# OpenDriveLab/ViDAR

Measured on AMD Instinct MI355X. Metric: train samples/sec (6-cam->BEV step), higher is better.
Workload: dtype f32

## Files before the change

### include/vidar_hip.h

```cpp
#ifndef VIDAR_HIP_H_
#define VIDAR_HIP_H_

#include <stddef.h>
#include <stdint.h>

#ifdef __cplusplus
extern "C" {
#endif

#define VIDAR_ERR_BAD_ARG (-22)

int vidar_abi_version(void);
int vidar_marker(int id, void* stream);

int vidar_set_deterministic(int on);
int vidar_get_deterministic(void);

int vidar_dvr_max_d(void);

int vidar_dvr_render_forward_f32(const float* sigma, const float* origin, const float* points,
                                 const float* tindex, float* pred_dist ,
                                 float* gt_dist , int N, int M, int T, int TO, int Z, int Y,
                                 int X, int train_phase, void* stream);

// ... 175 lines not shown
                            void* workspace, size_t workspace_bytes, void* stream);
int vidar_ray_occupancy_cam_f32(const float* sigma, const float* pix2vox, float* hit, float* free_,
                                int F, int C, int Hs, int Ws, float u0, float v0, float du, float dv,
                                int Z, int Y, int X, int K, float step,
                                void* workspace, size_t workspace_bytes, void* stream);

#define VIDAR_GEMM_F32 0
#define VIDAR_GEMM_BF16X3 1
#define VIDAR_GEMM_K_MAJOR 0
#define VIDAR_GEMM_MN_MAJOR 1
int vidar_gemm_f32(const float* A, int64_t lda, int a_layout, const float* B, int64_t ldb, int b_layout, float* C,
                   int64_t ldc, int M, int N, int K, int batch, int64_t strideA, int64_t strideB, int64_t strideC,
                   const float* scale, const float* shift, int vec_axis, const float* residual, int64_t ldr,
                   int64_t strideR, int relu, int precision, int reduce, float* a_rowsum, void* workspace,
                   size_t workspace_bytes, void* stream);
int vidar_gemm_splits(int M, int N, int K, int batch, int precision, int reduce);
size_t vidar_gemm_workspace_bytes(int M, int N, int K, int batch, int precision, int reduce);
int vidar_gemm_set_variant(int variant);

int vidar_dcn_set_variant(int variant);
int vidar_dcn_im2col_f32(const float* x, const float* offset, const float* mask, float* cols, int N,
                         int C, int H, int W, int Ho, int Wo, int kh, int kw, int stride, int pad,
                         int dil, void* stream);
int vidar_dcn_col2im_det_workspace_bytes(int N, int C, int H, int W, int64_t* bytes);
int vidar_dcn_col2im_f32(const float* grad_cols, const float* x, const float* offset,
                         const float* mask, float* grad_x, float* grad_offset, float* grad_mask,
                         int N, int C, int H, int W, int Ho, int Wo, int kh, int kw, int stride,
                         int pad, int dil, void* workspace, size_t workspace_bytes, void* stream);
size_t vidar_dcn_col2im_workspace_bytes(int N, int H, int W, int Ho, int Wo, int kh, int kw);

// ... 65 lines not shown
```

### vidar_amd/_lib.py

```python
from __future__ import annotations

import ctypes
import os
from pathlib import Path

_PKG = Path(__file__).resolve().parent
LIB_PATH = _PKG / "libvidar_hip.so"
_lib = None
BAD_ARG = -22


class VidarHipError(RuntimeError):
    pass


def lib() -> ctypes.CDLL:
    global _lib
    if _lib is None:
        import torch
        if not LIB_PATH.exists():
            raise VidarHipError(
                f"{LIB_PATH} not found: build it with `python -m vidar_amd.build` "
                f"(or __graft_entry__.build()); vidar_amd has no CPU fallback")
        _lib = declare(ctypes.CDLL(str(LIB_PATH)))
# ... 65 lines not shown
    "vidar_ray_gumbel_fwd_f32": "i 7p 6i f p",
    "vidar_ray_gumbel_bwd_f32": "i 7p 6i f p z p",
    "vidar_ray_argmax_f32": "i 6p 6i f p",
    "vidar_ray_dist_fwd_f32": "i 9p 6i f p",
    "vidar_ray_dist_bwd_f32": "i 7p 6i f p z p",
    "vidar_ray_max_k": "i",
    "vidar_ray_force_streamed": "i i",
    "vidar_ray_argmax_cam_f32": "i 3p 4i 4f 4i f p",
    "vidar_cam_rays_f32": "i 3p 4i 4f p",
    "vidar_ray_stats_f32": "i 7p 6i f p",
    "vidar_ray_stats_cam_f32": "i 4p 4i 4f 4i f p",
    "vidar_ray_occupancy_workspace_bytes": "i 4i p",
    "vidar_ray_occupancy_f32": "i 6p 6i f p z p",
    "vidar_ray_occupancy_cam_f32": "i 4p 4i 4f 4i f p z p",
    "vidar_gemm_f32": "i p l i p l i p l 4i 3l 2p i p 2l 3i 2p z p",
    "vidar_gemm_splits": "i 6i",
    "vidar_gemm_workspace_bytes": "z 6i",
    "vidar_gemm_set_variant": "i i",
    "vidar_dcn_set_variant": "i i",
    "vidar_dcn_im2col_f32": "i 4p 11i p",
    "vidar_dcn_col2im_f32": "i 7p 11i p z p",
    "vidar_dcn_col2im_workspace_bytes": "z 7i",
    "vidar_dcn_col2im_det_workspace_bytes": "i 4i p",
    "vidar_conv3x3_few_workspace_bytes": "z i",
    "vidar_conv3x3_few_f32": "i 4p 5i p z p",
    "vidar_affine_act_fwd_f32": "i 5p 4i p",
    "vidar_stem_bn_relu_pool_f32": "i 4p 4i p",
    "vidar_affine_act_bwd_f32": "i 5p 4i p",
    "vidar_dcnv3_set_variant": "i i",
    "vidar_dcnv3_forward_f32": "i 4p 13i f p",
# ... 107 lines not shown
```

### vidar_amd/csrc/gemm_mfma.hip

```cpp
#include <hip/hip_runtime.h>

#include <stdint.h>

#include <type_traits>

#include "vidar_hip.h"
#include "vidar_common.h"

namespace {

typedef __bf16 bf16x8 __attribute__((ext_vector_type(8)));
typedef __bf16 bf16x2 __attribute__((ext_vector_type(2)));
typedef float f32x16 __attribute__((ext_vector_type(16)));
typedef float f32x2 __attribute__((ext_vector_type(2)));
typedef float f32x4 __attribute__((ext_vector_type(4)));
typedef float f32x4u __attribute__((ext_vector_type(4), aligned(4)));
typedef uint32_t u32x4 __attribute__((ext_vector_type(4)));
typedef uint32_t u32x2 __attribute__((ext_vector_type(2)));

constexpr int BM = 128, BN = 128, THREADS = 256;
constexpr int BK = 32;
constexpr int MN_STRIDE = 128 + 8;
template <int PREC>
struct Geo {
// ... 6 lines not shown
constexpr int LAY_K = 0, LAY_MN = 1;

struct GemmArgs {
  const float* A; const float* B; float* C;
  int64_t lda, ldb, ldc, sA, sB, sC;
  int M, N, K;
  int splits, k_chunk;
  int slabs;
  const float* scale; const float* shift; int vec_axis;
  const float* residual; int64_t ldr, sR;
  int relu;
  int tiles_m, tiles_n, m_fastest;
  int total;
  float* a_rowsum;
  float* rowsum_ws;
};

struct Lane {
  int wm, wn, l31, h;
  __device__ __forceinline__ Lane(int tid, int wave) : wm((wave >> 1) * 64), wn((wave & 1) * 64), l31(tid & 31), h((tid & 63) >> 5) {}
  __device__ __forceinline__ explicit Lane(int tid) : Lane(tid, tid >> 6) {}
  __device__ __forceinline__ uint32_t voff(uint32_t ld) const { return (uint32_t)(((wm + 4 * h) * ld + wn + l31) * 4); }
};

__device__ __forceinline__ void zero_acc(f32x16 (&acc)[2][2]) {
#pragma unroll
  for (int i = 0; i < 2; ++i)
#pragma unroll
    for (int j = 0; j < 2; ++j)
#pragma unroll
      for (int r = 0; r < 16; ++r) acc[i][j][r] = 0.0f;
// ... 103 lines not shown
      *(u32x4*)(img + u * MN_STRIDE + cq) = hi;
      *(u32x4*)(img + Geo<PREC>::IMG_DWORDS + u * MN_STRIDE + cq) = lo;
    }
  } else {
#pragma unroll
    for (int i = 0; i < 4; ++i) {
      const int item = tid + 256 * i;
      *(u32x4*)(img + (item >> 5) * MN_STRIDE + (item & 31) * 4) = __builtin_bit_cast(u32x4, s.v[i >> 1][i & 1]);
    }
  }
}
template <int PREC, int ALAY, int BLAY>
__device__ __forceinline__ void stage_pair(const Staged& sa, const Staged& sb, uint32_t* imgA, uint32_t* imgB, int tid) {
  stage<PREC, ALAY>(sa, imgA, tid);
  stage<PREC, BLAY>(sb, imgB, tid);
}

template <int PREC, int LAY>
__device__ __forceinline__ u32x4 frag(const uint32_t* img, int row, int s, int h) {
  if (LAY == LAY_K) {
    if (PREC == PREC_BF16X3)
      return *(const u32x4*)(img + row * Geo<PREC>::KM_STRIDE + (((2 * s + h) ^ ((row >> 2) & 3)) << 2));
    return *(const u32x4*)(img + row * Geo<PREC>::KM_STRIDE + 8 * s + 4 * h);
  }
  u32x4 f;
  const uint32_t* p = img + (8 * s + 4 * h) * MN_STRIDE + row;
#pragma unroll
  for (int j = 0; j < 4; ++j) f[j] = p[j * MN_STRIDE];
  return f;
}
// ... 70 lines not shown
          }
    } else {
#pragma unroll
      for (int u = 0; u < 4; ++u)
#pragma unroll
        for (int i = 0; i < 2; ++i)
#pragma unroll
          for (int j = 0; j < 2; ++j) {
            const f32x4 bf = __builtin_bit_cast(f32x4, fb[j][0]), af = __builtin_bit_cast(f32x4, fa[i][0]);
            acc[i][j] = __builtin_amdgcn_mfma_f32_32x32x2f32(af[u], bf[u], acc[i][j], 0, 0, 0);
          }
    }
  }
}

template <int PREC, int ALAY, int BLAY>
__device__ __forceinline__ void mainloop(f32x16 (&acc)[2][2], Staged& sa, Staged& sb, const GemmArgs& g, const Tile& T,
                                         int kstop, uint32_t* imgA, uint32_t* imgB, int tid, uint32_t voa, uint32_t vob,
                                         f32x4& rowsum, bool want_rowsum) {
  const Lane c(tid);
  for (int k0 = T.kbeg; k0 < kstop; k0 += BK) {
    if (ALAY == LAY_MN && want_rowsum) add_rowsum(rowsum, sa);
    stage_pair<PREC, ALAY, BLAY>(sa, sb, imgA, imgB, tid);
    __syncthreads();
    if (k0 + BK < T.kend) fetch<PREC, ALAY, BLAY>(sa, sb, g, T, k0 + BK, tid, voa, vob);
    mma_step<PREC, ALAY, BLAY>(acc, imgA, imgB, c);
    __syncthreads();
  }
}

__device__ __forceinline__ float finish(float acc, float sc, float sh, float rs, int relu) {
  float y = acc * sc + sh + rs;
  if (relu && !(y > 0.0f)) y = 0.0f;
  return y;
}

template <bool RAGGED_M>
__device__ __forceinline__ void epilogue_impl(const f32x16 (&acc)[2][2], const GemmArgs& g, const Tile& T, int tid) {
  const Lane c(tid);
  const int m0 = T.m0, n0 = T.n0;
  float* C; int64_t ldc;
  if (g.slabs) { C = g.C + (int64_t)T.z * g.M * g.N; ldc = g.N; }
  else { C = g.C + (int64_t)T.batch * g.sC; ldc = g.ldc; }
  const bool epi = !g.slabs;
  const bool by_n = epi && g.vec_axis == 0, by_m = epi && g.vec_axis == 1;
  const int rows_left = g.M - m0, cols_left = g.N - n0;
  const int mleft = rows_left - c.wm - 4 * c.h;
  const __amdgpu_buffer_rsrc_t rsC = window_rsrc(C + (int64_t)m0 * ldc + n0, ldc, rows_left, cols_left);
  const uint32_t voC = c.voff((uint32_t)ldc);
  const bool has_res = epi && g.residual != nullptr;
  const float* Rp = has_res ? g.residual + (int64_t)T.batch * g.sR + (int64_t)m0 * g.ldr + n0 : C;
  const __amdgpu_buffer_rsrc_t rsR = window_rsrc(Rp, g.ldr, rows_left, cols_left, has_res);
// ... 13 lines not shown
    for (int i = 0; i < 2; ++i) {
#pragma unroll
      for (int r0 = 0; r0 < 16; r0 += 8) {
        float sc[8], sh[8], rs[8];
#pragma unroll
        for (int r = 0; r < 8; ++r) {
          const int row = 32 * i + (r & 3) + 8 * ((r0 + r) >> 2);
          sc[r] = m_scale ? ld4(rsS, voM, (uint32_t)(row * 4)) : sn;
          sh[r] = m_shift ? ld4(rsH, voM, (uint32_t)(row * 4)) : bn;
          rs[r] = has_res ? ld4(rsR, voR, (uint32_t)((row * (uint32_t)g.ldr + 32 * j) * 4)) : 0.0f;
        }
#pragma unroll
        for (int r = 0; r < 8; ++r) {
          const int row = 32 * i + (r & 3) + 8 * ((r0 + r) >> 2);
          float y = acc[i][j][r0 + r];
          if (epi) y = finish(y, sc[r], sh[r], rs[r], g.relu);
          if (!RAGGED_M || row < mleft)
            __builtin_amdgcn_raw_buffer_store_b32(__builtin_bit_cast(uint32_t, y), rsC, voC,
                                                    (uint32_t)((row * (uint32_t)ldc + 32 * j) * 4), 0);
        }
      }
    }
  }
}

__device__ __forceinline__ void epilogue(const f32x16 (&acc)[2][2], const GemmArgs& g, const Tile& T, int tid) {
  if (g.M - T.m0 >= BM) epilogue_impl<false>(acc, g, T, tid);
  else epilogue_impl<true>(acc, g, T, tid);
}

constexpr int TAB_DWORDS = 2 * (BM + BM);

__device__ __forceinline__ void lds_barrier() { asm volatile("s_waitcnt lgkmcnt(0)\n\ts_barrier" ::: "memory"); }

__device__ __forceinline__ bool piped_tile(const GemmArgs& g, const Tile& T) {
  return !g.slabs && (g.vec_axis == 1 || (g.scale == nullptr && g.shift == nullptr)) && g.M - T.m0 >= BM &&
         g.N - T.n0 >= BN && T.kbeg < T.kend;
}

__device__ __forceinline__ float table_value(const GemmArgs& g, const Tile& T, int tid) {
  const float* v = tid < BM ? g.scale : g.shift;
  float x = tid < BM ? 1.0f : 0.0f;
  if (v != nullptr) x = v[T.m0 + (tid & (BM - 1))];
  return x;
}

template <int ALAY, int BLAY>
__device__ __forceinline__ void last_step_stage(const Staged& sa, const Staged& sb, uint32_t* imgA, uint32_t* imgB,
                                                float* tab, float tabv, int tid) {
  stage_pair<PREC_F32, ALAY, BLAY>(sa, sb, imgA, imgB, tid);
  tab[tid] = tabv;
  __syncthreads();
}

template <int ALAY, int BLAY>
__device__ __forceinline__ void last_step_piped(f32x16 (&acc)[2][2], const GemmArgs& g, const Tile& T, const uint32_t* imgA,
                                                const uint32_t* imgB, const float* tab, int tid0) {
  constexpr int PREC = PREC_F32;
  int tid = tid0;
  asm volatile("" : "+v"(tid));
  const Lane c(tid);
  const __amdgpu_buffer_rsrc_t rsC =
      window_rsrc(g.C + (int64_t)T.batch * g.sC + (int64_t)T.m0 * g.ldc + T.n0, g.ldc, BM, BN);
  const uint32_t ldc = (uint32_t)g.ldc, ldr = (uint32_t)g.ldr;
// ... 26 lines not shown
        if (sub < 4) acc[i][j] = __builtin_amdgcn_mfma_f32_32x32x2f32(af[u], bf[u], acc[i][j], 0, 0, 0);
        if (sub > 0) {
          const int r = 4 * s + u;
          const int prow = 32 * pi + 8 * s + u;
          const float y = finish(acc[pi][pj][r], tsc[prow], tsh[prow], rs[r], g.relu);
          __builtin_amdgcn_raw_buffer_store_b32(__builtin_bit_cast(uint32_t, y), rsC, voC, (uint32_t)((prow * ldc + 32 * pj) * 4), 0);
          if (sub < 4) rs[r] = ld4(rsR, voRz, (uint32_t)(((32 * i + 8 * s + u) * ldr + 32 * j) * rb));
        }
      }
      __builtin_amdgcn_sched_barrier(0);
    }
    if (sub == 3) lds_barrier();
  }
}

template <int PREC, int ALAY, int BLAY>
__global__ __launch_bounds__(THREADS, 3) void gemm_mfma_kernel(GemmArgs g) {
  constexpr int IMGS = (PREC == PREC_BF16X3) ? 2 : 1;
  constexpr int IMGS_DWORDS = 2 * IMGS * Geo<PREC>::IMG_DWORDS;
  __shared__ __attribute__((aligned(16))) uint32_t lds[IMGS_DWORDS + (PREC == PREC_F32 && ALAY == LAY_K ? TAB_DWORDS : 0)];
  uint32_t* imgA = lds;
  uint32_t* imgB = lds + IMGS * Geo<PREC>::IMG_DWORDS;
  const int tid = threadIdx.x;
  const uint32_t voa = voff<PREC, ALAY>(g.lda, tid), vob = voff<PREC, BLAY>(g.ldb, tid);
  Staged sa, sb;
  int t = blockIdx.x;
  if (t >= g.total) return;
  Tile cur = decode_tile<PREC, ALAY, BLAY>(g, t);
  if (cur.kbeg < cur.kend) fetch<PREC, ALAY, BLAY>(sa, sb, g, cur, cur.kbeg, tid, voa, vob);
  for (int parity = 0;; parity ^= 1) {
    f32x16 acc[2][2];
    zero_acc(acc);
    f32x4 rowsum = {0.f, 0.f, 0.f, 0.f};
    const bool want_rowsum = ALAY == LAY_MN && g.a_rowsum != nullptr && cur.n0 == 0;
    const int tn = t + (int)gridDim.x;
    const bool more = tn < g.total;
    constexpr bool PIPED = PREC == PREC_F32 && ALAY == LAY_K;
    const bool piped = PIPED && piped_tile(g, cur);
    float tabv = 0.0f;
    if (piped) tabv = table_value(g, cur, tid);
    const int kstop = piped ? cur.kbeg + (cur.kend - cur.kbeg - 1) / BK * BK : cur.kend;
    mainloop<PREC, ALAY, BLAY>(acc, sa, sb, g, cur, kstop, imgA, imgB, tid, voa, vob, rowsum, want_rowsum);
    float* tab = reinterpret_cast<float*>(lds) + IMGS_DWORDS + parity * (TAB_DWORDS / 2);
    if constexpr (PIPED) {
      if (piped) last_step_stage<ALAY, BLAY>(sa, sb, imgA, imgB, tab, tabv, tid);
    }
    if (want_rowsum) {
      float* red = reinterpret_cast<float*>(lds);
      const int quad = tid & 31, part = tid >> 5;
      *(f32x4*)(red + (part * 32 + quad) * 4) = rowsum;
      __syncthreads();
      if (tid < BM) {
        float sum = 0.f;
#pragma unroll
        for (int p8 = 0; p8 < 8; ++p8) sum += red[(p8 * 32 + (tid >> 2)) * 4 + (tid & 3)];
        if (cur.m0 + tid < g.M) g.rowsum_ws[(int64_t)cur.z * g.M + cur.m0 + tid] = sum;
      }
      __syncthreads();
    }
    if (more) {
      const Tile nxt = decode_tile<PREC, ALAY, BLAY>(g, tn);
      if (nxt.kbeg < nxt.kend) fetch<PREC, ALAY, BLAY>(sa, sb, g, nxt, nxt.kbeg, tid, voa, vob);
    }
    if constexpr (PIPED) {
      if (piped) last_step_piped<ALAY, BLAY>(acc, g, cur, imgA, imgB, tab, tid);
      else epilogue(acc, g, cur, tid);
    } else {
      epilogue(acc, g, cur, tid);
    }
    if (!more) break;
    cur = decode_tile<PREC, ALAY, BLAY>(g, tn);
    t = tn;
  }
}

constexpr int WS_THREADS = 512;

template <int PREC, int ALAY, int BLAY>
struct Cursor {
  int t;
  int k0;
  Tile T;
  __device__ __forceinline__ void start(const GemmArgs& g, int t0) {
// ... 108 lines not shown
}

int g_gemm_variant = 0;

template <class F>
void with_layouts(int a_layout, int b_layout, F f) {
  using K = std::integral_constant<int, LAY_K>;
  using MN = std::integral_constant<int, LAY_MN>;
  if (a_layout == LAY_K && b_layout == LAY_K) f(K{}, K{});
  else if (a_layout == LAY_K) f(K{}, MN{});
  else if (b_layout == LAY_K) f(MN{}, K{});
  else f(MN{}, MN{});
}

template <int PREC>
void launch(const GemmArgs& g, int a_layout, int b_layout, bool ws, int grid, hipStream_t st) {
  with_layouts(a_layout, b_layout, [&](auto a, auto b) {
    constexpr int ALAY = decltype(a)::value, BLAY = decltype(b)::value;
    if (ws) hipLaunchKernelGGL((gemm_mfma_ws_kernel<PREC, ALAY, BLAY>), dim3(grid), dim3(WS_THREADS), 0, st, g);
    else hipLaunchKernelGGL((gemm_mfma_kernel<PREC, ALAY, BLAY>), dim3(grid), dim3(THREADS), 0, st, g);
  });
}

int num_cus() {
  static int cached[64] = {0};
  int dev = 0;
  if (hipGetDevice(&dev) != hipSuccess || dev < 0 || dev >= 64) return 256;
  if (cached[dev] == 0) {
    hipDeviceProp_t prop;
    cached[dev] = (hipGetDeviceProperties(&prop, dev) == hipSuccess && prop.multiProcessorCount > 0)
                      ? prop.multiProcessorCount : 256;
  }
  return cached[dev];
}
// ... 5 lines not shown
  if (s > max_s) s = max_s;
  if (s < 1) s = 1;
  if (s > 256) s = 256;
  return s;
}

size_t slab_workspace_bytes(int Z, int M, int N, bool rowsum) {
  return (size_t)Z * ((size_t)M * N + (rowsum ? M : 0)) * sizeof(float);
}

int resident_grid(int total, int per_cu) {
  const int resident = num_cus() * per_cu / 8 * 8;
  return total > resident ? resident : total;
}

}

extern "C" {

int vidar_gemm_set_variant(int variant) {
  const int prev = g_gemm_variant;
  g_gemm_variant = (variant < 0 || variant > 2) ? 0 : variant;
  return prev;
}

int vidar_gemm_splits(int M, int N, int K, int batch, int precision, int reduce) {
  if (!reduce) return 1;
  return pick_splits(M, N, K, batch);
}

size_t vidar_gemm_workspace_bytes(int M, int N, int K, int batch, int precision, int reduce) {
  if (!reduce) return 0;
  const int Z = batch * pick_splits(M, N, K, batch);
  if (reduce == 1) return Z > 1 ? slab_workspace_bytes(Z, M, N, false) : 0;
  return slab_workspace_bytes(Z, M, N, true);
}

int vidar_gemm_f32(const float* A, int64_t lda, int a_layout, const float* B, int64_t ldb, int b_layout, float* C,
                   int64_t ldc, int M, int N, int K, int batch, int64_t strideA, int64_t strideB, int64_t strideC,
                   const float* scale, const float* shift, int vec_axis, const float* residual, int64_t ldr,
                   int64_t strideR, int relu, int precision, int reduce, float* a_rowsum, void* workspace,
                   size_t workspace_bytes, void* stream) {
  VIDAR_ENTER();
  if (a_rowsum != nullptr && !(reduce && a_layout == LAY_MN)) return VIDAR_ERR_BAD_ARG;
  if (A == nullptr || B == nullptr || C == nullptr || M <= 0 || N <= 0 || K <= 0 || batch <= 0) return VIDAR_ERR_BAD_ARG;
  if ((a_layout != LAY_K && a_layout != LAY_MN) || (b_layout != LAY_K && b_layout != LAY_MN)) return VIDAR_ERR_BAD_ARG;
  if (precision != PREC_F32 && precision != PREC_BF16X3) return VIDAR_ERR_BAD_ARG;
  if (vec_axis != 0 && vec_axis != 1) return VIDAR_ERR_BAD_ARG;
  if (lda < (a_layout == LAY_K ? K : M) || ldb < (b_layout == LAY_K ? K : N) || ldc < N) return VIDAR_ERR_BAD_ARG;
  if (residual != nullptr && (ldr < N || ldr >= (1 << 22))) return VIDAR_ERR_BAD_ARG;
  if (ldc >= (1 << 22)) return VIDAR_ERR_BAD_ARG;
  if (lda >= (1 << 22) || ldb >= (1 << 22)) return VIDAR_ERR_BAD_ARG;
  if ((a_layout == LAY_MN && (int64_t)K * lda >= (1LL << 29)) || (b_layout == LAY_MN && (int64_t)K * ldb >= (1LL << 29)))
    return VIDAR_ERR_BAD_ARG;
  hipStream_t st = (hipStream_t)stream;
  GemmArgs g;
  g.A = A; g.B = B; g.C = C;
  g.lda = lda; g.ldb = ldb; g.ldc = ldc; g.sA = strideA; g.sB = strideB; g.sC = strideC;
  g.M = M; g.N = N; g.K = K;
  g.scale = scale; g.shift = shift; g.vec_axis = vec_axis; g.residual = residual; g.ldr = ldr; g.sR = strideR;
  g.relu = relu;
  g.tiles_m = (M + BM - 1) / BM; g.tiles_n = (N + BN - 1) / BN;
  g.m_fastest = M < N;
  g.splits = reduce ? pick_splits(M, N, K, batch) : 1;
  g.k_chunk = ((K + g.splits - 1) / g.splits + BK - 1) / BK * BK;
  const int Z = batch * g.splits;
  g.slabs = (reduce && (Z > 1 || a_rowsum != nullptr)) ? 1 : 0;
  g.a_rowsum = a_rowsum;
  g.rowsum_ws = nullptr;
  if ((int64_t)g.tiles_m * g.tiles_n * Z > 0x3fffffff) return VIDAR_ERR_BAD_ARG;
  g.total = g.tiles_m * g.tiles_n * Z;
  if (reduce && (strideC != 0 || strideR != 0) && batch > 1) return VIDAR_ERR_BAD_ARG;
  if (g.slabs) {
    if (workspace == nullptr || workspace_bytes < slab_workspace_bytes(Z, M, N, a_rowsum != nullptr)) return VIDAR_ERR_BAD_ARG;
    g.rowsum_ws = a_rowsum ? (float*)workspace + (size_t)Z * M * N : nullptr;
  }
  const bool ws = g_gemm_variant >= 1 && a_rowsum == nullptr;
  const int grid = resident_grid(g.total, ws ? g_gemm_variant : 3);
  GemmArgs tiles = g;
  if (g.slabs) tiles.C = (float*)workspace;
  if (precision == PREC_BF16X3) launch<PREC_BF16X3>(tiles, a_layout, b_layout, ws, grid, st);
  else launch<PREC_F32>(tiles, a_layout, b_layout, ws, grid, st);
  if (g.slabs) {
    const int64_t total = (int64_t)M * N;
    int blocks = (int)((total / 4 + 1 + 63) / 64);
    if (blocks > 4096) blocks = 4096;
    hipLaunchKernelGGL(gemm_slab_reduce_kernel, dim3(blocks), dim3(256), 0, st, (const float*)workspace, Z, g);
  }
  return vidar_last_error();
}

}
```

### vidar_amd/gemm.py

```python
from __future__ import annotations

import contextlib
import os

import torch

from ._lib import lib, check, ptr, stream_of, workspace, TIMER
from . import deterministic

F32, BF16X3 = 0, 1
K_MAJOR, MN_MAJOR = 0, 1
_MODES = ("lib", "auto", "f32", "bf16x3")
_mode = os.environ.get("VIDAR_GEMM", "auto")
if _mode not in _MODES:
    raise ValueError(f"VIDAR_GEMM={_mode!r}: expected one of {_MODES}")


def mode() -> str:
    return _mode


def set_mode(m: str) -> str:
    global _mode
    if m not in _MODES:
# ... 46 lines not shown
def _operand(t, layout, contraction, what):
    if not t.is_cuda:
        raise RuntimeError(f"vidar_gemm: {what} must be a CUDA tensor (no CPU path)")
    if t.dtype != torch.float32:
        raise TypeError(f"vidar_gemm: {what} must be float32, got {t.dtype}")
    if operand_ok(t, layout, contraction):
        return t
    c = t.contiguous()
    if not operand_ok(c, layout, contraction):
        raise ValueError(f"vidar_gemm: {what} {tuple(t.shape)} exceeds the kernel's addressing range "
                         f"(leading dimension < 2^22, contraction x leading dimension < 2^29)")
    return c


def gemm_raw(A, lda, a_layout, B, ldb, b_layout, C, ldc, M, N, K, *, batch=1, sA=0, sB=0, sC=0, scale=None, shift=None,
             vec_axis=0, residual=None, ldr=0, sR=0, relu=False, precision=F32, reduce=False, a_rowsum=None, name="gemm"):
    L = lib()
    ws, ws_ptr, nbytes = workspace(L.vidar_gemm_workspace_bytes, M, N, K, batch, precision, 2 if a_rowsum is not None else 1,
                                   like=C) if reduce else (None, None, 0)
    flops = 2.0 * M * N * K * batch
    with TIMER.span(name, flops):
        check(L.vidar_gemm_f32(ptr(A), lda, a_layout, ptr(B), ldb, b_layout, ptr(C), ldc, M, N, K, batch, sA, sB, sC,
                               ptr(scale), ptr(shift), vec_axis, ptr(residual), ldr, sR, bool(relu), precision,
                               bool(reduce), ptr(a_rowsum), ws_ptr, nbytes, stream_of(C)),
              "vidar_gemm_f32")
    return C


def linear_forward(x2, weight, bias=None, relu=False, precision=F32):
    M, K = x2.shape
    N = weight.shape[0]
    x2 = _operand(x2, K_MAJOR, K, "x"); weight = _operand(weight, K_MAJOR, K, "weight")
    y = torch.empty((M, N), dtype=torch.float32, device=x2.device)
    if M == 0:
        return y
# ... 66 lines not shown
        if ctx.needs_input_grad[1]:
            gw = linear_grad_weight(g2, x2, precision, with_bias=want_b)
            if want_b:
                gw, gb = gw
        elif want_b:
            gb = _colsum(g2)
        return gx, gw, gb, None, None


def linear(x, weight, bias=None, relu=False, m: str | None = None):
    n = weight.shape[0]
    y = MfmaLinear.apply(x.reshape(-1, x.shape[-1]), weight, bias, bool(relu), precision_of(m))
    return y.view(*x.shape[:-1], n)


def conv_forward(w2, x3, scale=None, shift=None, residual=None, relu=False, precision=F32):
    _f32c(w2, "weight"); _f32c(x3, "x")
    Bn, Ci, HW = x3.shape
    Co = w2.shape[0]
    y = torch.empty((Bn, Co, HW), dtype=torch.float32, device=x3.device)
    if residual is not None:
        assert residual.shape == y.shape and residual.is_contiguous()
    return gemm_raw(w2, w2.stride(0), K_MAJOR, x3, x3.stride(1), MN_MAJOR, y, HW, Co, HW, Ci, batch=Bn, sA=0,
                    sB=x3.stride(0), sC=Co * HW, scale=scale, shift=shift, vec_axis=1, residual=residual, ldr=HW,
                    sR=Co * HW, relu=relu, precision=precision, name="gemm_conv_fwd")


def conv_grad_input(w2, g3, precision=F32):
    _f32c(w2, "weight"); _f32c(g3, "grad_out")
    Bn, Co, HW = g3.shape
    Ci = w2.shape[1]
    gx = torch.empty((Bn, Ci, HW), dtype=torch.float32, device=g3.device)
    return gemm_raw(w2, w2.stride(0), MN_MAJOR, g3, g3.stride(1), MN_MAJOR, gx, HW, Ci, HW, Co, batch=Bn, sA=0,
                    sB=g3.stride(0), sC=Ci * HW, precision=precision, name="gemm_conv_dx")


def conv_grad_weight(g3, x3, precision=F32, scale=None):
    _f32c(g3, "grad_out"); _f32c(x3, "x")
    Bn, Co, HW = g3.shape
    Ci = x3.shape[1]
    gw = torch.empty((Co, Ci), dtype=torch.float32, device=g3.device)
    return gemm_raw(g3, g3.stride(1), K_MAJOR, x3, x3.stride(1), K_MAJOR, gw, Ci, Co, Ci, HW, batch=Bn,
                    sA=g3.stride(0), sB=x3.stride(0), scale=scale, vec_axis=1, precision=precision, reduce=True,
                    name="gemm_conv_dw")
```

### vidar_amd/plugin/backbones.py

```python
from __future__ import annotations

import ctypes
import math
import os

import torch
import torch.nn as nn
import torch.nn.functional as F
from torch.autograd import Function
from torch.autograd.function import once_differentiable

from .registry import BACKBONES, NECKS
from .._lib import lib, check, ptr, stream_of, workspace, TIMER
from .. import gemm as G
from .. import deterministic


def dcn_col2im(grad_cols, x, offset, mask, kh, kw, stride, pad, dil, Ho, Wo, gather=True):
    N, C, H, W = x.shape
    gx = torch.empty_like(x); goff = torch.empty_like(offset); gm = torch.empty_like(mask)
    if deterministic.sync():
        nbytes = ctypes.c_int64(0)
        check(lib().vidar_dcn_col2im_det_workspace_bytes(N, C, H, W, ctypes.addressof(nbytes)), "dcn_col2im")
        nbytes = nbytes.value
# ... 271 lines not shown
        return gx, gw


_SHORTCUT_ACCUMULATE = os.environ.get("VIDAR_SHORTCUT_ACCUMULATE", "1") != "0"


def conv1x1_with_identity_ok(conv, x):
    return (_SHORTCUT_ACCUMULATE and isinstance(conv, Conv1x1) and conv.gemm_form(x) and conv.stride == (1, 1)
            and conv.bias is None and x.dtype == torch.float32 and conv.weight.dtype == torch.float32
            and x.requires_grad and torch.is_grad_enabled() and not torch.is_autocast_enabled() and x.is_contiguous())


class _Conv1x1BNAct(Function):

    @staticmethod
    def forward(ctx, x, weight, scale, shift, residual, relu, precision):
        x = x.float().contiguous()
        N, C, H, W = x.shape
        Cout = weight.shape[0]
        res = residual.float().contiguous().view(N, Cout, H * W) if residual is not None else None
        y = G.conv_forward(weight.reshape(Cout, C), x.view(N, C, H * W), scale, shift, res, relu, precision)
        ctx.save_for_backward(x, weight, scale, y if relu else None)
        ctx.cfg = (relu, residual is not None, precision)
        return y.view(N, Cout, H, W)

    @staticmethod
    @once_differentiable
    def backward(ctx, gy):
        x, weight, scale, y = ctx.saved_tensors
        relu, has_res, precision = ctx.cfg
        N, C, H, W = x.shape
        Cout = weight.shape[0]
        gy = gy.float().contiguous().view(N, Cout, H * W)
        gz, gres = _affine_act_backward(gy, y if relu else gy, scale, relu, has_res)
        gx = G.conv_grad_input(weight.reshape(Cout, C), gz, precision).view(N, C, H, W) if ctx.needs_input_grad[0] else None
        gw = G.conv_grad_weight(gz, x.view(N, C, H * W), precision).view_as(weight) if ctx.needs_input_grad[1] else None
        return gx, gw, None, None, (gres.view(N, Cout, H, W) if has_res else None), None, None


def _fuses_1x1(conv, bn, x, residual, hw, m):
    fuse = G.own_kernels(m) or (m == "auto" and residual is not None and _AUTO_FUSE_RES)
    in_range = 0 < hw < (1 << 22) and max(conv.in_channels, conv.out_channels) * hw < (1 << 29)
    return (fuse and x.is_cuda and not bn.weight.requires_grad and conv.bias is None and conv.kernel_size == (1, 1)
            and conv.padding == (0, 0) and conv.groups == 1 and in_range)


def conv1x1_bn_act(conv, bn, x, residual=None, relu=False, presampled=False):
    if presampled:
        return _conv1x1_bn_act_presampled(conv, bn, x, residual, relu)
    m = G.mode()
    hw = ((x.shape[2] - 1) // conv.stride[0] + 1) * ((x.shape[3] - 1) // conv.stride[1] + 1) if x.dim() == 4 else 0
    if not _fuses_1x1(conv, bn, x, residual, hw, m):
        return bn(conv(x), residual=residual, relu=relu)
    if conv.stride != (1, 1):
        x = x[:, :, ::conv.stride[0], ::conv.stride[1]]
    scale, shift = bn._scale_shift()
    return _Conv1x1BNAct.apply(x, conv.weight, scale, shift, residual, bool(relu), G.precision_of(m))


def _conv1x1_bn_act_presampled(conv, bn, xs, residual, relu):
    m = G.mode()
    if not _fuses_1x1(conv, bn, xs, residual, xs.shape[2] * xs.shape[3] if xs.dim() == 4 else 0, m):
        return bn(conv(xs, presampled=True), residual=residual, relu=relu)
    scale, shift = bn._scale_shift()
    return _Conv1x1BNAct.apply(xs, conv.weight, scale, shift, residual, bool(relu), G.precision_of(m))


_SHARE_SUBSAMPLE = os.environ.get("VIDAR_SHARE_SUBSAMPLE", "1") != "0"


class Bottleneck(nn.Module):
    expansion = 4

    def __init__(self, inplanes, planes, stride=1, downsample=None, style="caffe", dcn=None, bn_grad=False):
        super().__init__()
        s1, s2 = (stride, 1) if style == "caffe" else (1, stride)
        self.conv1 = Conv1x1(inplanes, planes, 1, stride=s1, bias=False)
        self.bn1 = FrozenBN(planes, bn_grad)
        if dcn is not None:
            self.conv2 = ModulatedDeformConv2dPack(planes, planes, 3, stride=s2, padding=1, dilation=1,
# ... 24 lines not shown
                                                                            x.shape[2] * x.shape[3], G.mode()):
                out, identity = _Conv1x1Identity.apply(x, self.conv1.weight)
                return self._tail(self.bn1(out, relu=True), identity)
        elif len(self.downsample) == 2 and isinstance(self.downsample[1], FrozenBN):
            identity = conv1x1_bn_act(self.downsample[0], self.downsample[1], x)
        else:
            identity = self.downsample(x)
        out = conv1x1_bn_act(self.conv1, self.bn1, x, relu=True)
        return self._tail(out, identity)

    def _tail(self, out, identity):
        if (isinstance(self.conv2, ModulatedDeformConv2dPack) and G.own_kernels() and out.is_cuda
                and not self.bn2.weight.requires_grad):
            out = self.conv2(out, bn=self.bn2, relu=True)
        else:
            out = self.bn2(self.conv2(out), relu=True)
        return conv1x1_bn_act(self.conv3, self.bn3, out, residual=identity, relu=True)


@BACKBONES.register_module()
class ResNet(nn.Module):
    arch = {50: (3, 4, 6, 3), 101: (3, 4, 23, 3), 152: (3, 8, 36, 3)}

    def __init__(self, depth=101, num_stages=4, out_indices=(0, 1, 2, 3), frozen_stages=-1,
                 norm_cfg=dict(type="BN", requires_grad=True), norm_eval=True, style="pytorch", dcn=None,
                 stage_with_dcn=(False, False, False, False), strides=(1, 2, 2, 2), in_channels=3,
                 base_channels=64, init_cfg=None, pretrained=None, **kwargs):
        super().__init__()
        if dcn is not None and dcn.get("type") != "DCNv2":
            raise NotImplementedError(dcn)
        bn_grad = norm_cfg.get("requires_grad", True)
# ... 95 lines not shown
```

Before: 2.932.

## Fuse bn2 affine+ReLU into conv3 GEMM operand load and backward gating

Adds a fused GEMM entry point that applies a per-channel scale/shift plus ReLU to the B operand as it is staged into LDS. It also adds a gated epilogue that recomputes the ReLU mask from the saved pre-activation in the input-gradient GEMM. Bottleneck blocks with a frozen bn2 and no DCN now feed raw conv2 output straight into conv3. This skips materialising the bn2 activation tensor in forward and the separate ReLU-backward pass. In exchange it adds per-tile transform arithmetic in the mainloop and an extra kernel instantiation, and it is excluded for 64-plane blocks when training.

Result: no change. 2.950, median of 6 (+0.6%).

```diff
diff --git a/include/vidar_hip.h b/include/vidar_hip.h
--- a/include/vidar_hip.h
+++ b/include/vidar_hip.h
@@ -213,6 +213,12 @@
                    const float* scale, const float* shift, int vec_axis, const float* residual, int64_t ldr,
                    int64_t strideR, int relu, int precision, int reduce, float* a_rowsum, void* workspace,
                    size_t workspace_bytes, void* stream);
+int vidar_gemm_fused_f32(const float* A, int64_t lda, int a_layout, const float* B, int64_t ldb, int b_layout, float* C,
+                         int64_t ldc, int M, int N, int K, int batch, int64_t strideA, int64_t strideB, int64_t strideC,
+                         const float* scale, const float* shift, int vec_axis, const float* residual, int64_t ldr,
+                         int64_t strideR, int relu, int precision, int reduce, float* a_rowsum, void* workspace,
+                         size_t workspace_bytes, const float* b_scale, const float* b_shift, const float* gate,
+                         int64_t ldg, int64_t strideG, void* stream);
 int vidar_gemm_splits(int M, int N, int K, int batch, int precision, int reduce);
 size_t vidar_gemm_workspace_bytes(int M, int N, int K, int batch, int precision, int reduce);
 int vidar_gemm_set_variant(int variant);
diff --git a/vidar_amd/_lib.py b/vidar_amd/_lib.py
--- a/vidar_amd/_lib.py
+++ b/vidar_amd/_lib.py
@@ -103,6 +103,7 @@
     "vidar_ray_occupancy_f32": "i 6p 6i f p z p",
     "vidar_ray_occupancy_cam_f32": "i 4p 4i 4f 4i f p z p",
     "vidar_gemm_f32": "i p l i p l i p l 4i 3l 2p i p 2l 3i 2p z p",
+    "vidar_gemm_fused_f32": "i p l i p l i p l 4i 3l 2p i p 2l 3i 2p z 3p 2l p",
     "vidar_gemm_splits": "i 6i",
     "vidar_gemm_workspace_bytes": "z 6i",
     "vidar_gemm_set_variant": "i i",
diff --git a/vidar_amd/csrc/gemm_mfma.hip b/vidar_amd/csrc/gemm_mfma.hip
--- a/vidar_amd/csrc/gemm_mfma.hip
+++ b/vidar_amd/csrc/gemm_mfma.hip
@@ -44,7 +44,11 @@
   int total;
   float* a_rowsum;
   float* rowsum_ws;
+  const float* b_scale; const float* b_shift;
 };
+
+constexpr int XF_NONE = 0, XF_BIN = 1, XF_GATE = 2;
+constexpr int BTAB = 512;
 
 struct Lane {
   int wm, wn, l31, h;
@@ -178,6 +182,17 @@
 __device__ __forceinline__ void stage_pair(const Staged& sa, const Staged& sb, uint32_t* imgA, uint32_t* imgB, int tid) {
   stage<PREC, ALAY>(sa, imgA, tid);
   stage<PREC, BLAY>(sb, imgB, tid);
+}
+
+template <int BLAY>
+__device__ __forceinline__ void transform_b(Staged& s, const float* tab, int base, int tid) {
+  const int first = base + (BLAY == LAY_K ? 32 * (tid >> 6) + (tid & 63) / KM_LPR : (tid >> 5));
+#pragma unroll
+  for (int i = 0; i < Staged::CH * 2; ++i) {
+    const float sc = tab[first + 8 * i], sh = tab[BTAB + first + 8 * i];
+#pragma unroll
+    for (int j = 0; j < 4; ++j) s.v[i >> 1][i & 1][j] = fmaxf(__builtin_fmaf(s.v[i >> 1][i & 1][j], sc, sh), 0.0f);
+  }
 }
 
 template <int PREC, int LAY>
@@ -278,13 +293,14 @@
   }
 }
 
-template <int PREC, int ALAY, int BLAY>
+template <int PREC, int ALAY, int BLAY, int XF>
 __device__ __forceinline__ void mainloop(f32x16 (&acc)[2][2], Staged& sa, Staged& sb, const GemmArgs& g, const Tile& T,
                                          int kstop, uint32_t* imgA, uint32_t* imgB, int tid, uint32_t voa, uint32_t vob,
-                                         f32x4& rowsum, bool want_rowsum) {
+                                         f32x4& rowsum, bool want_rowsum, const float* btab) {
   const Lane c(tid);
   for (int k0 = T.kbeg; k0 < kstop; k0 += BK) {
     if (ALAY == LAY_MN && want_rowsum) add_rowsum(rowsum, sa);
+    if (XF == XF_BIN) transform_b<BLAY>(sb, btab, BLAY == LAY_MN ? k0 : T.n0, tid);
     stage_pair<PREC, ALAY, BLAY>(sa, sb, imgA, imgB, tid);
     __syncthreads();
     if (k0 + BK < T.kend) fetch<PREC, ALAY, BLAY>(sa, sb, g, T, k0 + BK, tid, voa, vob);
@@ -299,7 +315,7 @@
   return y;
 }
 
-template <bool RAGGED_M>
+template <bool RAGGED_M, bool GATE>
 __device__ __forceinline__ void epilogue_impl(const f32x16 (&acc)[2][2], const GemmArgs& g, const Tile& T, int tid) {
   const Lane c(tid);
   const int m0 = T.m0, n0 = T.n0;
@@ -343,7 +359,8 @@
         for (int r = 0; r < 8; ++r) {
           const int row = 32 * i + (r & 3) + 8 * ((r0 + r) >> 2);
           float y = acc[i][j][r0 + r];
-          if (epi) y = finish(y, sc[r], sh[r], rs[r], g.relu);
+          if (GATE) y = (__builtin_fmaf(rs[r], sc[r], sh[r]) > 0.0f ? y : 0.0f) * sc[r];
+          else if (epi) y = finish(y, sc[r], sh[r], rs[r], g.relu);
           if (!RAGGED_M || row < mleft)
             __builtin_amdgcn_raw_buffer_store_b32(__builtin_bit_cast(uint32_t, y), rsC, voC,
                                                     (uint32_t)((row * (uint32_t)ldc + 32 * j) * 4), 0);
@@ -353,9 +370,10 @@
   }
 }
 
+template <bool GATE = false>
 __device__ __forceinline__ void epilogue(const f32x16 (&acc)[2][2], const GemmArgs& g, const Tile& T, int tid) {
-  if (g.M - T.m0 >= BM) epilogue_impl<false>(acc, g, T, tid);
-  else epilogue_impl<true>(acc, g, T, tid);
+  if (g.M - T.m0 >= BM) epilogue_impl<false, GATE>(acc, g, T, tid);
+  else epilogue_impl<true, GATE>(acc, g, T, tid);
 }
 
 constexpr int TAB_DWORDS = 2 * (BM + BM);
@@ -374,9 +392,10 @@
   return x;
 }
 
-template <int ALAY, int BLAY>
-__device__ __forceinline__ void last_step_stage(const Staged& sa, const Staged& sb, uint32_t* imgA, uint32_t* imgB,
-                                                float* tab, float tabv, int tid) {
+template <int ALAY, int BLAY, int XF>
+__device__ __forceinline__ void last_step_stage(const Staged& sa, Staged& sb, uint32_t* imgA, uint32_t* imgB,
+                                                float* tab, float tabv, int tid, const float* btab, int bbase) {
+  if (XF == XF_BIN) transform_b<BLAY>(sb, btab, bbase, tid);
   stage_pair<PREC_F32, ALAY, BLAY>(sa, sb, imgA, imgB, tid);
   tab[tid] = tabv;
   __syncthreads();
@@ -433,11 +452,15 @@
   }
 }
 
-template <int PREC, int ALAY, int BLAY>
+template <int PREC, int ALAY, int BLAY, int XF = XF_NONE>
 __global__ __launch_bounds__(THREADS, 3) void gemm_mfma_kernel(GemmArgs g) {
+  static_assert(XF == XF_NONE || (PREC == PREC_F32 && (XF == XF_BIN ? ALAY == LAY_K : ALAY == LAY_MN && BLAY == LAY_MN)),
+                "XF_BIN: fp32 with a K-major A; XF_GATE: fp32 with both operands MN-major");
   constexpr int IMGS = (PREC == PREC_BF16X3) ? 2 : 1;
   constexpr int IMGS_DWORDS = 2 * IMGS * Geo<PREC>::IMG_DWORDS;
-  __shared__ __attribute__((aligned(16))) uint32_t lds[IMGS_DWORDS + (PREC == PREC_F32 && ALAY == LAY_K ? TAB_DWORDS : 0)];
+  constexpr int TABS_DWORDS = PREC == PREC_F32 && ALAY == LAY_K ? TAB_DWORDS : 0;
+  __shared__ __attribute__((aligned(16))) uint32_t lds[IMGS_DWORDS + TABS_DWORDS + (XF == XF_BIN ? 2 * BTAB : 0)];
+  float* btab = reinterpret_cast<float*>(lds) + IMGS_DWORDS + TABS_DWORDS;
   uint32_t* imgA = lds;
   uint32_t* imgB = lds + IMGS * Geo<PREC>::IMG_DWORDS;
   const int tid = threadIdx.x;
@@ -447,6 +470,14 @@
   if (t >= g.total) return;
   Tile cur = decode_tile<PREC, ALAY, BLAY>(g, t);
   if (cur.kbeg < cur.kend) fetch<PREC, ALAY, BLAY>(sa, sb, g, cur, cur.kbeg, tid, voa, vob);
+  if constexpr (XF == XF_BIN) {
+    const int nvec = BLAY == LAY_MN ? g.K : g.N;
+    for (int i = tid; i < BTAB; i += THREADS) {
+      btab[i] = i < nvec ? g.b_scale[i] : 0.0f;
+      btab[BTAB + i] = i < nvec ? g.b_shift[i] : 0.0f;
+    }
+    __syncthreads();
+  }
   for (int parity = 0;; parity ^= 1) {
     f32x16 acc[2][2];
     zero_acc(acc);
@@ -459,10 +490,10 @@
     float tabv = 0.0f;
     if (piped) tabv = table_value(g, cur, tid);
     const int kstop = piped ? cur.kbeg + (cur.kend - cur.kbeg - 1) / BK * BK : cur.kend;
-    mainloop<PREC, ALAY, BLAY>(acc, sa, sb, g, cur, kstop, imgA, imgB, tid, voa, vob, rowsum, want_rowsum);
+    mainloop<PREC, ALAY, BLAY, XF>(acc, sa, sb, g, cur, kstop, imgA, imgB, tid, voa, vob, rowsum, want_rowsum, btab);
     float* tab = reinterpret_cast<float*>(lds) + IMGS_DWORDS + parity * (TAB_DWORDS / 2);
     if constexpr (PIPED) {
-      if (piped) last_step_stage<ALAY, BLAY>(sa, sb, imgA, imgB, tab, tabv, tid);
+      if (piped) last_step_stage<ALAY, BLAY, XF>(sa, sb, imgA, imgB, tab, tabv, tid, btab, BLAY == LAY_MN ? kstop : cur.n0);
     }
     if (want_rowsum) {
       float* red = reinterpret_cast<float*>(lds);
@@ -485,7 +516,7 @@
       if (piped) last_step_piped<ALAY, BLAY>(acc, g, cur, imgA, imgB, tab, tid);
       else epilogue(acc, g, cur, tid);
     } else {
-      epilogue(acc, g, cur, tid);
+      epilogue<XF == XF_GATE>(acc, g, cur, tid);
     }
     if (!more) break;
     cur = decode_tile<PREC, ALAY, BLAY>(g, tn);
@@ -624,10 +655,16 @@
 }
 
 template <int PREC>
-void launch(const GemmArgs& g, int a_layout, int b_layout, bool ws, int grid, hipStream_t st) {
+void launch(const GemmArgs& g, int a_layout, int b_layout, bool ws, int xf, int grid, hipStream_t st) {
   with_layouts(a_layout, b_layout, [&](auto a, auto b) {
     constexpr int ALAY = decltype(a)::value, BLAY = decltype(b)::value;
-    if (ws) hipLaunchKernelGGL((gemm_mfma_ws_kernel<PREC, ALAY, BLAY>), dim3(grid), dim3(WS_THREADS), 0, st, g);
+    if (xf == XF_BIN) {
+      if constexpr (PREC == PREC_F32 && ALAY == LAY_K)
+        hipLaunchKernelGGL((gemm_mfma_kernel<PREC, ALAY, BLAY, XF_BIN>), dim3(grid), dim3(THREADS), 0, st, g);
+    } else if (xf == XF_GATE) {
+      if constexpr (PREC == PREC_F32 && ALAY == LAY_MN && BLAY == LAY_MN)
+        hipLaunchKernelGGL((gemm_mfma_kernel<PREC, ALAY, BLAY, XF_GATE>), dim3(grid), dim3(THREADS), 0, st, g);
+    } else if (ws) hipLaunchKernelGGL((gemm_mfma_ws_kernel<PREC, ALAY, BLAY>), dim3(grid), dim3(WS_THREADS), 0, st, g);
     else hipLaunchKernelGGL((gemm_mfma_kernel<PREC, ALAY, BLAY>), dim3(grid), dim3(THREADS), 0, st, g);
   });
 }
@@ -663,33 +700,11 @@
   return total > resident ? resident : total;
 }
 
-}
-
-extern "C" {
-
-int vidar_gemm_set_variant(int variant) {
-  const int prev = g_gemm_variant;
-  g_gemm_variant = (variant < 0 || variant > 2) ? 0 : variant;
-  return prev;
-}
-
-int vidar_gemm_splits(int M, int N, int K, int batch, int precision, int reduce) {
-  if (!reduce) return 1;
-  return pick_splits(M, N, K, batch);
-}
-
-size_t vidar_gemm_workspace_bytes(int M, int N, int K, int batch, int precision, int reduce) {
-  if (!reduce) return 0;
-  const int Z = batch * pick_splits(M, N, K, batch);
-  if (reduce == 1) return Z > 1 ? slab_workspace_bytes(Z, M, N, false) : 0;
-  return slab_workspace_bytes(Z, M, N, true);
-}
-
-int vidar_gemm_f32(const float* A, int64_t lda, int a_layout, const float* B, int64_t ldb, int b_layout, float* C,
-                   int64_t ldc, int M, int N, int K, int batch, int64_t strideA, int64_t strideB, int64_t strideC,
-                   const float* scale, const float* shift, int vec_axis, const float* residual, int64_t ldr,
-                   int64_t strideR, int relu, int precision, int reduce, float* a_rowsum, void* workspace,
-                   size_t workspace_bytes, void* stream) {
+int gemm_call(const float* A, int64_t lda, int a_layout, const float* B, int64_t ldb, int b_layout, float* C, int64_t ldc,
+              int M, int N, int K, int batch, int64_t strideA, int64_t strideB, int64_t strideC, const float* scale,
+              const float* shift, int vec_axis, const float* residual, int64_t ldr, int64_t strideR, int relu, int precision,
+              int reduce, float* a_rowsum, void* workspace, size_t workspace_bytes, const float* b_scale,
+              const float* b_shift, const float* gate, int64_t ldg, int64_t strideG, void* stream) {
   VIDAR_ENTER();
   if (a_rowsum != nullptr && !(reduce && a_layout == LAY_MN)) return VIDAR_ERR_BAD_ARG;
   if (A == nullptr || B == nullptr || C == nullptr || M <= 0 || N <= 0 || K <= 0 || batch <= 0) return VIDAR_ERR_BAD_ARG;
@@ -699,6 +714,15 @@
   if (lda < (a_layout == LAY_K ? K : M) || ldb < (b_layout == LAY_K ? K : N) || ldc < N) return VIDAR_ERR_BAD_ARG;
   if (residual != nullptr && (ldr < N || ldr >= (1 << 22))) return VIDAR_ERR_BAD_ARG;
   if (ldc >= (1 << 22)) return VIDAR_ERR_BAD_ARG;
+  const bool bin = b_scale != nullptr || b_shift != nullptr;
+  if (bin && (b_scale == nullptr || b_shift == nullptr || precision != PREC_F32 || a_layout != LAY_K || gate != nullptr ||
+              (b_layout == LAY_MN ? K : N) > BTAB))
+    return VIDAR_ERR_BAD_ARG;
+  if (gate != nullptr && (precision != PREC_F32 || a_layout != LAY_MN || b_layout != LAY_MN || reduce || scale == nullptr ||
+                          shift == nullptr || vec_axis != 1 || residual != nullptr || relu || ldg < N || ldg >= (1 << 22)))
+    return VIDAR_ERR_BAD_ARG;
+  const int xf = bin ? XF_BIN : gate != nullptr ? XF_GATE : XF_NONE;
+  if (gate != nullptr) { residual = gate; ldr = ldg; strideR = strideG; }
   if (lda >= (1 << 22) || ldb >= (1 << 22)) return VIDAR_ERR_BAD_ARG;
   if ((a_layout == LAY_MN && (int64_t)K * lda >= (1LL << 29)) || (b_layout == LAY_MN && (int64_t)K * ldb >= (1LL << 29)))
     return VIDAR_ERR_BAD_ARG;
@@ -717,6 +741,7 @@
   g.slabs = (reduce && (Z > 1 || a_rowsum != nullptr)) ? 1 : 0;
   g.a_rowsum = a_rowsum;
   g.rowsum_ws = nullptr;
+  g.b_scale = b_scale; g.b_shift = b_shift;
   if ((int64_t)g.tiles_m * g.tiles_n * Z > 0x3fffffff) return VIDAR_ERR_BAD_ARG;
   g.total = g.tiles_m * g.tiles_n * Z;
   if (reduce && (strideC != 0 || strideR != 0) && batch > 1) return VIDAR_ERR_BAD_ARG;
@@ -724,12 +749,12 @@
     if (workspace == nullptr || workspace_bytes < slab_workspace_bytes(Z, M, N, a_rowsum != nullptr)) return VIDAR_ERR_BAD_ARG;
     g.rowsum_ws = a_rowsum ? (float*)workspace + (size_t)Z * M * N : nullptr;
   }
-  const bool ws = g_gemm_variant >= 1 && a_rowsum == nullptr;
+  const bool ws = g_gemm_variant >= 1 && a_rowsum == nullptr && xf == XF_NONE;
   const int grid = resident_grid(g.total, ws ? g_gemm_variant : 3);
   GemmArgs tiles = g;
   if (g.slabs) tiles.C = (float*)workspace;
-  if (precision == PREC_BF16X3) launch<PREC_BF16X3>(tiles, a_layout, b_layout, ws, grid, st);
-  else launch<PREC_F32>(tiles, a_layout, b_layout, ws, grid, st);
+  if (precision == PREC_BF16X3) launch<PREC_BF16X3>(tiles, a_layout, b_layout, ws, XF_NONE, grid, st);
+  else launch<PREC_F32>(tiles, a_layout, b_layout, ws, xf, grid, st);
   if (g.slabs) {
     const int64_t total = (int64_t)M * N;
     int blocks = (int)((total / 4 + 1 + 63) / 64);
@@ -740,3 +765,46 @@
 }
 
 }
+
+extern "C" {
+
+int vidar_gemm_set_variant(int variant) {
+  const int prev = g_gemm_variant;
+  g_gemm_variant = (variant < 0 || variant > 2) ? 0 : variant;
+  return prev;
+}
+
+int vidar_gemm_splits(int M, int N, int K, int batch, int precision, int reduce) {
+  if (!reduce) return 1;
+  return pick_splits(M, N, K, batch);
+}
+
+size_t vidar_gemm_workspace_bytes(int M, int N, int K, int batch, int precision, int reduce) {
+  if (!reduce) return 0;
+  const int Z = batch * pick_splits(M, N, K, batch);
+  if (reduce == 1) return Z > 1 ? slab_workspace_bytes(Z, M, N, false) : 0;
+  return slab_workspace_bytes(Z, M, N, true);
+}
+
+int vidar_gemm_f32(const float* A, int64_t lda, int a_layout, const float* B, int64_t ldb, int b_layout, float* C,
+                   int64_t ldc, int M, int N, int K, int batch, int64_t strideA, int64_t strideB, int64_t strideC,
+                   const float* scale, const float* shift, int vec_axis, const float* residual, int64_t ldr,
+                   int64_t strideR, int relu, int precision, int reduce, float* a_rowsum, void* workspace,
+                   size_t workspace_bytes, void* stream) {
+  return gemm_call(A, lda, a_layout, B, ldb, b_layout, C, ldc, M, N, K, batch, strideA, strideB, strideC, scale, shift,
+                   vec_axis, residual, ldr, strideR, relu, precision, reduce, a_rowsum, workspace, workspace_bytes, nullptr,
+                   nullptr, nullptr, 0, 0, stream);
+}
+
+int vidar_gemm_fused_f32(const float* A, int64_t lda, int a_layout, const float* B, int64_t ldb, int b_layout, float* C,
+                         int64_t ldc, int M, int N, int K, int batch, int64_t strideA, int64_t strideB, int64_t strideC,
+                         const float* scale, const float* shift, int vec_axis, const float* residual, int64_t ldr,
+                         int64_t strideR, int relu, int precision, int reduce, float* a_rowsum, void* workspace,
+                         size_t workspace_bytes, const float* b_scale, const float* b_shift, const float* gate,
+                         int64_t ldg, int64_t strideG, void* stream) {
+  return gemm_call(A, lda, a_layout, B, ldb, b_layout, C, ldc, M, N, K, batch, strideA, strideB, strideC, scale, shift,
+                   vec_axis, residual, ldr, strideR, relu, precision, reduce, a_rowsum, workspace, workspace_bytes, b_scale,
+                   b_shift, gate, ldg, strideG, stream);
+}
+
+}
diff --git a/vidar_amd/gemm.py b/vidar_amd/gemm.py
--- a/vidar_amd/gemm.py
+++ b/vidar_amd/gemm.py
@@ -84,11 +84,20 @@
 
 
 def gemm_raw(A, lda, a_layout, B, ldb, b_layout, C, ldc, M, N, K, *, batch=1, sA=0, sB=0, sC=0, scale=None, shift=None,
-             vec_axis=0, residual=None, ldr=0, sR=0, relu=False, precision=F32, reduce=False, a_rowsum=None, name="gemm"):
+             vec_axis=0, residual=None, ldr=0, sR=0, relu=False, precision=F32, reduce=False, a_rowsum=None, name="gemm",
+             b_scale=None, b_shift=None, gate=None, ldg=0, sG=0):
     L = lib()
     ws, ws_ptr, nbytes = workspace(L.vidar_gemm_workspace_bytes, M, N, K, batch, precision, 2 if a_rowsum is not None else 1,
                                    like=C) if reduce else (None, None, 0)
     flops = 2.0 * M * N * K * batch
+    if b_scale is not None or gate is not None:
+        with TIMER.span(name, flops):
+            check(L.vidar_gemm_fused_f32(ptr(A), lda, a_layout, ptr(B), ldb, b_layout, ptr(C), ldc, M, N, K, batch, sA, sB,
+                                         sC, ptr(scale), ptr(shift), vec_axis, ptr(residual), ldr, sR, bool(relu),
+                                         precision, bool(reduce), ptr(a_rowsum), ws_ptr, nbytes, ptr(b_scale),
+                                         ptr(b_shift), ptr(gate), ldg, sG, stream_of(C)),
+                  "vidar_gemm_fused_f32")
+        return C
     with TIMER.span(name, flops):
         check(L.vidar_gemm_f32(ptr(A), lda, a_layout, ptr(B), ldb, b_layout, ptr(C), ldc, M, N, K, batch, sA, sB, sC,
                                ptr(scale), ptr(shift), vec_axis, ptr(residual), ldr, sR, bool(relu), precision,
@@ -185,7 +194,10 @@
     return y.view(*x.shape[:-1], n)
 
 
-def conv_forward(w2, x3, scale=None, shift=None, residual=None, relu=False, precision=F32):
+IN_AFFINE_MAX = 512
+
+
+def conv_forward(w2, x3, scale=None, shift=None, residual=None, relu=False, precision=F32, in_scale=None, in_shift=None):
     _f32c(w2, "weight"); _f32c(x3, "x")
     Bn, Ci, HW = x3.shape
     Co = w2.shape[0]
@@ -194,23 +206,29 @@
         assert residual.shape == y.shape and residual.is_contiguous()
     return gemm_raw(w2, w2.stride(0), K_MAJOR, x3, x3.stride(1), MN_MAJOR, y, HW, Co, HW, Ci, batch=Bn, sA=0,
                     sB=x3.stride(0), sC=Co * HW, scale=scale, shift=shift, vec_axis=1, residual=residual, ldr=HW,
-                    sR=Co * HW, relu=relu, precision=precision, name="gemm_conv_fwd")
-
-
-def conv_grad_input(w2, g3, precision=F32):
+                    sR=Co * HW, relu=relu, precision=precision, name="gemm_conv_fwd", b_scale=in_scale, b_shift=in_shift)
+
+
+def conv_grad_input(w2, g3, precision=F32, gate=None, scale=None, shift=None):
     _f32c(w2, "weight"); _f32c(g3, "grad_out")
     Bn, Co, HW = g3.shape
     Ci = w2.shape[1]
     gx = torch.empty((Bn, Ci, HW), dtype=torch.float32, device=g3.device)
+    if gate is not None:
+        _f32c(gate, "gate")
+        assert gate.shape == gx.shape and scale is not None and shift is not None
+        return gemm_raw(w2, w2.stride(0), MN_MAJOR, g3, g3.stride(1), MN_MAJOR, gx, HW, Ci, HW, Co, batch=Bn, sA=0,
+                        sB=g3.stride(0), sC=Ci * HW, scale=scale, shift=shift, vec_axis=1, precision=precision,
+                        name="gemm_conv_dx", gate=gate, ldg=gate.stride(1), sG=gate.stride(0))
     return gemm_raw(w2, w2.stride(0), MN_MAJOR, g3, g3.stride(1), MN_MAJOR, gx, HW, Ci, HW, Co, batch=Bn, sA=0,
                     sB=g3.stride(0), sC=Ci * HW, precision=precision, name="gemm_conv_dx")
 
 
-def conv_grad_weight(g3, x3, precision=F32, scale=None):
+def conv_grad_weight(g3, x3, precision=F32, scale=None, in_scale=None, in_shift=None):
     _f32c(g3, "grad_out"); _f32c(x3, "x")
     Bn, Co, HW = g3.shape
     Ci = x3.shape[1]
     gw = torch.empty((Co, Ci), dtype=torch.float32, device=g3.device)
     return gemm_raw(g3, g3.stride(1), K_MAJOR, x3, x3.stride(1), K_MAJOR, gw, Ci, Co, Ci, HW, batch=Bn,
                     sA=g3.stride(0), sB=x3.stride(0), scale=scale, vec_axis=1, precision=precision, reduce=True,
-                    name="gemm_conv_dw")
+                    name="gemm_conv_dw", b_scale=in_scale, b_shift=in_shift)
diff --git a/vidar_amd/plugin/backbones.py b/vidar_amd/plugin/backbones.py
--- a/vidar_amd/plugin/backbones.py
+++ b/vidar_amd/plugin/backbones.py
@@ -309,28 +309,32 @@
 class _Conv1x1BNAct(Function):
 
     @staticmethod
-    def forward(ctx, x, weight, scale, shift, residual, relu, precision):
+    def forward(ctx, x, weight, scale, shift, residual, relu, precision, in_scale=None, in_shift=None):
         x = x.float().contiguous()
         N, C, H, W = x.shape
         Cout = weight.shape[0]
         res = residual.float().contiguous().view(N, Cout, H * W) if residual is not None else None
-        y = G.conv_forward(weight.reshape(Cout, C), x.view(N, C, H * W), scale, shift, res, relu, precision)
-        ctx.save_for_backward(x, weight, scale, y if relu else None)
+        y = G.conv_forward(weight.reshape(Cout, C), x.view(N, C, H * W), scale, shift, res, relu, precision,
+                           in_scale, in_shift)
+        ctx.save_for_backward(x, weight, scale, y if relu else None, in_scale, in_shift)
         ctx.cfg = (relu, residual is not None, precision)
         return y.view(N, Cout, H, W)
 
     @staticmethod
     @once_differentiable
     def backward(ctx, gy):
-        x, weight, scale, y = ctx.saved_tensors
+        x, weight, scale, y, in_scale, in_shift = ctx.saved_tensors
         relu, has_res, precision = ctx.cfg
         N, C, H, W = x.shape
         Cout = weight.shape[0]
         gy = gy.float().contiguous().view(N, Cout, H * W)
         gz, gres = _affine_act_backward(gy, y if relu else gy, scale, relu, has_res)
-        gx = G.conv_grad_input(weight.reshape(Cout, C), gz, precision).view(N, C, H, W) if ctx.needs_input_grad[0] else None
-        gw = G.conv_grad_weight(gz, x.view(N, C, H * W), precision).view_as(weight) if ctx.needs_input_grad[1] else None
-        return gx, gw, None, None, (gres.view(N, Cout, H, W) if has_res else None), None, None
+        x3 = x.view(N, C, H * W)
+        gate = dict(gate=x3, scale=in_scale, shift=in_shift) if in_scale is not None else {}
+        gx = G.conv_grad_input(weight.reshape(Cout, C), gz, precision, **gate).view(N, C, H, W) if ctx.needs_input_grad[0] else None
+        gw = G.conv_grad_weight(gz, x3, precision, in_scale=in_scale, in_shift=in_shift).view_as(weight) \
+            if ctx.needs_input_grad[1] else None
+        return gx, gw, None, None, (gres.view(N, Cout, H, W) if has_res else None), None, None, None, None
 
 
 def _fuses_1x1(conv, bn, x, residual, hw, m):
@@ -359,6 +363,21 @@
         return bn(conv(xs, presampled=True), residual=residual, relu=relu)
     scale, shift = bn._scale_shift()
     return _Conv1x1BNAct.apply(xs, conv.weight, scale, shift, residual, bool(relu), G.precision_of(m))
+
+
+_BN2_FUSE_FWD_ONLY = frozenset({64})
+
+
+def _fuses_bn2(block, z, identity):
+    planes = block.conv3.in_channels
+    m = G.mode()
+    if planes in _BN2_FUSE_FWD_ONLY and torch.is_grad_enabled() and (z.requires_grad or block.conv3.weight.requires_grad):
+        return False
+    return (os.environ.get("VIDAR_FUSE_BN2", "1") != "0" and z.is_cuda and z.dtype == torch.float32 and z.dim() == 4
+            and not torch.is_autocast_enabled() and not block.bn2.weight.requires_grad
+            and block.conv3.weight.dtype == torch.float32 and G.precision_of(m) == G.F32
+            and block.conv3.stride == (1, 1) and _fuses_1x1(block.conv3, block.bn3, z, identity, z.shape[2] * z.shape[3], m)
+            and planes % 32 == 0 and planes <= G.IN_AFFINE_MAX)
 
 
 _SHARE_SUBSAMPLE = os.environ.get("VIDAR_SHARE_SUBSAMPLE", "1") != "0"
@@ -413,7 +432,12 @@
                 and not self.bn2.weight.requires_grad):
             out = self.conv2(out, bn=self.bn2, relu=True)
         else:
-            out = self.bn2(self.conv2(out), relu=True)
+            out = self.conv2(out)
+            if _fuses_bn2(self, out, identity):
+                in_scale, in_shift = self.bn2._scale_shift()
+                scale, shift = self.bn3._scale_shift()
+                return _Conv1x1BNAct.apply(out, self.conv3.weight, scale, shift, identity, True, G.F32, in_scale, in_shift)
+            out = self.bn2(out, relu=True)
         return conv1x1_bn_act(self.conv3, self.bn3, out, residual=identity, relu=True)
 
 
```
